# ubc-vision/RefTR

Measured on AMD Instinct MI355X. Metric: images/sec training step, RefCOCO R50 640x640 bs=8/GPU, higher is better.
Workload: dtype bf16; 1 GPU; RefCOCO-shaped REC train step, ResNet-50 + BERT-base + VL transformer 6+6, 640x640, batch 8/GPU, L=40, aux loss, dropout on, clip 0.1, AdamW (configs[1]); global_batch=8, batch_per_gpu=8, image_size=640, parallelism=dp1, launch=hipgraph

## Files before the change

reftr_amd/csrc/rt_qregion.hip:

```cpp
#include "rt_common.h"
#include "rt_ln_row.h"
#include "rt_loss_row.h"

namespace {

constexpr int QE = 256;
constexpr int QT = 1024;
constexpr int QH = QT / 256;
constexpr int QW = QT / 64;

__device__ __forceinline__ f32x4 ld4(const float* p) { return *reinterpret_cast<const f32x4*>(p); }
__device__ __forceinline__ void st4(float* p, const f32x4 v) { *reinterpret_cast<f32x4*>(p) = v; }
__device__ __forceinline__ void st4b(bf16_t* p, const f32x4 v) {
    bf16x4 b;
#pragma unroll
    for (int e = 0; e < 4; ++e) b[e] = (bf16_t)v[e];
    *reinterpret_cast<bf16x4*>(p) = b;
}

template <int MT, int K, typename XRow, typename Epi>
__device__ __forceinline__ void q_tile(const bf16_t* __restrict__ W, const int ldw, const int n0, const int nmax,
                                       XRow xrow, const int M, Epi epi) {
    const int lane = threadIdx.x & 63, li = lane & 15, lg = lane >> 4;
    int n = n0 + li; if (n >= nmax) n = nmax - 1;
    const bf16_t* wp = W + (size_t)n * ldw + lg * 8;
    const bf16_t* xp[MT];
    f32x4 acc[MT];
#pragma unroll
    for (int t = 0; t < MT; ++t) {
        int m = t * 16 + li; if (m >= M) m = M - 1;
        xp[t] = xrow(m) + lg * 8;
        acc[t] = f32x4{0.f, 0.f, 0.f, 0.f};
    }
    constexpr int KC = MT >= 3 ? 128 : (K < 256 ? K : 256), NK = KC / 32;
#pragma unroll
    for (int k0 = 0; k0 < K; k0 += KC) {
        bf16x8 a[NK], x[MT][NK];
#pragma unroll
        for (int i = 0; i < NK; ++i) a[i] = *reinterpret_cast<const bf16x8*>(wp + k0 + i * 32);
#pragma unroll
        for (int t = 0; t < MT; ++t)
#pragma unroll
            for (int i = 0; i < NK; ++i) x[t][i] = *reinterpret_cast<const bf16x8*>(xp[t] + k0 + i * 32);
        __builtin_amdgcn_sched_barrier(0);
#pragma unroll
        for (int i = 0; i < NK; ++i)
#pragma unroll
            for (int t = 0; t < MT; ++t)
                acc[t] = __builtin_amdgcn_mfma_f32_16x16x32_bf16(a[i], x[t][i], acc[t], 0, 0, 0);
        __builtin_amdgcn_sched_barrier(0);
    }
#pragma unroll
    for (int t = 0; t < MT; ++t) {
        const int m = t * 16 + li;
        if (m < M && n0 + lg * 4 < nmax) epi(m, n0 + lg * 4, acc[t]);
    }
}
constexpr int QLMAX = 96;
constexpr int QLD = QE + 8;
__device__ unsigned long long g_qtrace[3][24];
__device__ __forceinline__ void q_stamp(const int kernel, int& slot) {
    if (blockIdx.x == 0 && threadIdx.x == 0 && slot < 24) g_qtrace[kernel][slot] = __builtin_amdgcn_s_memrealtime();
    ++slot;
}
template <int K, typename Epi>
__device__ __forceinline__ void q_tile_lds(const bf16_t* __restrict__ W, const int ldw, const int n0, const int nmax,
                                           const bf16_t* Xs, const int ldx, const int M, const float* __restrict__ bias, Epi epi) {
    const int lane = threadIdx.x & 63, li = lane & 15, lg = lane >> 4;
    int n = n0 + li; if (n >= nmax) n = nmax - 1;
    const bf16_t* wp = W + (size_t)n * ldw + lg * 8;
    constexpr int NK = K / 32;
    bf16x8 a[NK];
#pragma unroll
    for (int i = 0; i < NK; ++i) a[i] = *reinterpret_cast<const bf16x8*>(wp + i * 32);
    const bool nok = n0 + lg * 4 < nmax;
    const f32x4 b4 = (bias && nok) ? ld4(bias + n0 + lg * 4) : f32x4{0.f, 0.f, 0.f, 0.f};
    for (int m0 = 0; m0 < M; m0 += 16) {
        int m = m0 + li; if (m >= M) m = M - 1;
        const bf16_t* xp = Xs + (size_t)m * ldx + lg * 8;
        f32x4 acc = f32x4{0.f, 0.f, 0.f, 0.f};
#pragma unroll
        for (int i = 0; i < NK; ++i)
            acc = __builtin_amdgcn_mfma_f32_16x16x32_bf16(a[i], *reinterpret_cast<const bf16x8*>(xp + i * 32), acc, 0, 0, 0);
        if (m0 + li < M && nok) epi(m0 + li, n0 + lg * 4, acc + b4);
    }
}
template <int K, typename XRow, typename Epi>
__device__ __forceinline__ void q_gemm(const bf16_t* __restrict__ W, const int ldw, const int N, XRow xrow, const int M, Epi epi,
                                       const int tile0 = 0, const int tile_stride = QW) {
    const int wave = threadIdx.x >> 6;
    const int ntiles = (N + 15) >> 4;
    for (int t = tile0 + wave; t < ntiles; t += tile_stride) {
        for (int m0 = 0; m0 < M; m0 += 48) {
            const int rows = min(48, M - m0);
            auto xr = [&](int m) { return xrow(m0 + m); };
            auto ep = [&](int m, int n, const f32x4& v) { epi(m0 + m, n, v); };
            if (rows <= 16)      q_tile<1, K>(W, ldw, t * 16, N, xr, rows, ep);
            else if (rows <= 32) q_tile<2, K>(W, ldw, t * 16, N, xr, rows, ep);
            else                 q_tile<3, K>(W, ldw, t * 16, N, xr, rows, ep);
        }
    }
}

__device__ __forceinline__ f32x4 q_ln(const float* x, const float* gamma, const float* beta, const float eps, const bool relu,
                                      float* mean_out, float* rstd_out) {
    const int lane = threadIdx.x & 63;
    const f32x4 v = ld4(x + lane * 4);
    float mean, rstd;
    rt_ln_stats<1>(&v, eps, mean, rstd);
    if (lane == 0) { *mean_out = mean; *rstd_out = rstd; }
    return rt_ln_affine(v, mean, rstd, ld4(gamma + lane * 4), ld4(beta + lane * 4), relu);
}
__device__ __forceinline__ f32x4 q_ln_bwd(const f32x4 d, const float* x, const float mean, const float rstd, const f32x4 gam, const f32x4 bet,
                                          const bool relu, f32x4& dg, f32x4& db) {
    f32x4 xh, g;
    float s1 = 0.f, s2 = 0.f;
    rt_ln_bwd_group(d, ld4(x + (threadIdx.x & 63) * 4), mean, rstd, gam, bet, relu, xh, g, s1, s2, dg, db);
    rt_ln_bwd_means<1>(s1, s2);
    return rt_ln_bwd_dx(g, xh, rstd, s1, s2);
}
__device__ __forceinline__ void ln_partials(float (*sm)[QE], const f32x4 dg, const f32x4 db, float* __restrict__ part) {
    const int lane = threadIdx.x & 63, wave = threadIdx.x >> 6;
    __syncthreads();
    st4(&sm[wave][lane * 4], dg); st4(&sm[QW + wave][lane * 4], db);
    __syncthreads();
    for (int c = threadIdx.x; c < 2 * QE; c += QT) {
        const int which = c / QE, col = c - which * QE;
        float a = 0.f;
#pragma unroll
        for (int w = 0; w < QW; ++w) a += sm[which * QW + w][col];
        part[((size_t)blockIdx.x * 2 + which) * QE + col] = a;
    }
}

__global__ __launch_bounds__(QT) void qenc_fwd_kernel(const rt_qenc_fwd_desc p) {
    int q_slot = 0; q_stamp(0, q_slot);
    __shared__ float sw[128];
    __shared__ float pw[128];
    __shared__ __attribute__((aligned(16))) bf16_t xs[QLMAX * QLD];
    __shared__ __attribute__((aligned(16))) float part[4][QE];
    const int b = blockIdx.x, lane = threadIdx.x & 63, wave = threadIdx.x >> 6;
    const int S = p.S, L = p.L, P = p.P;
    const bf16_t* mem16 = (const bf16_t*)p.mem16 + (size_t)b * S * QE;
    bf16_t* cls16 = (bf16_t*)p.cls16 + (size_t)b * QE;
    bf16_t* lang16 = (bf16_t*)p.lang16 + (size_t)b * L * QE;
    float* kq = p.kq + (size_t)b * QE;
    float* qs = p.qs + (size_t)b * L * QE;
    float* vs = p.vs + (size_t)b * L * QE;

    for (int i = threadIdx.x; i < L * (QE / 8); i += QT) {
        const int r = i / (QE / 8), c = (i % (QE / 8)) * 8;
        const bf16x8 v = *reinterpret_cast<const bf16x8*>(mem16 + (size_t)r * QE + c);
        *reinterpret_cast<bf16x8*>(xs + (size_t)r * QLD + c) = v;
        *reinterpret_cast<bf16x8*>(lang16 + (size_t)r * QE + c) = v;
        if (r == 0) *reinterpret_cast<bf16x8*>(cls16 + c) = v;
    }
    __syncthreads(); q_stamp(0, q_slot);
    for (int job = wave; job < 48; job += QW) {
        const int prod = job >> 4, t = job & 15;
        if (prod == 0)
            q_tile_lds<QE>((const bf16_t*)p.W1, QE, t * 16, QE, xs, QLD, 1, p.b1, [&](int, int n, const f32x4& v) { st4(kq + n, v); });
        else {
            float* out = prod == 1 ? qs : vs;
            q_tile_lds<QE>((const bf16_t*)(prod == 1 ? p.W2 : p.W3), QE, t * 16, QE, xs, QLD, L, prod == 1 ? p.b2 : p.b3,
                           [&](int m, int n, const f32x4& v) { st4(out + (size_t)m * QE + n, v); });
        }
    }
    __syncthreads(); q_stamp(0, q_slot);

    for (int l = wave; l < L; l += QW) {
        float s = 0.f;
        for (int d = lane; d < QE; d += 64) s += kq[d] * qs[(size_t)l * QE + d];
        s = rt_wave_sum(s);
        if (lane == 0) sw[l] = s;
    }
    __syncthreads(); q_stamp(0, q_slot);
    for (int j = 0; j < P; ++j) {
        const int r = b * P + j;
        const uint8_t* cm = p.ctx + (size_t)r * L;
        if (wave == 0) {
            const float s0 = lane < L ? (cm[lane] ? -INFINITY : sw[lane]) : -INFINITY;
            const float s1 = lane + 64 < L ? (cm[lane + 64] ? -INFINITY : sw[lane + 64]) : -INFINITY;
            const float m = rt_wave_max(fmaxf(s0, s1));
            const float e0 = lane < L ? __expf(s0 - m) : 0.f, e1 = lane + 64 < L ? __expf(s1 - m) : 0.f;
            const float tot = rt_wave_sum(e0) + rt_wave_sum(e1);
            const float inv = 1.f / tot;
            if (lane < L) { pw[lane] = e0 * inv; p.qw[(size_t)r * L + lane] = e0 * inv; }
            if (lane + 64 < L) { pw[lane + 64] = e1 * inv; p.qw[(size_t)r * L + lane + 64] = e1 * inv; }
        }
        __syncthreads();
        {
            const int qt = threadIdx.x >> 8, d = threadIdx.x & 255;
            const int per = (L + 3) >> 2, l0 = qt * per, l1 = min(L, l0 + per);
            float a = 0.f;
            for (int l = l0; l < l1; ++l) a += pw[l] * vs[(size_t)l * QE + d];
            part[qt][d] = a;
        }
        __syncthreads();
        if (threadIdx.x < QE) {
            const int d = threadIdx.x;
            ((bf16_t*)p.c16)[(size_t)r * QE + d] = (bf16_t)((part[0][d] + part[1][d]) + (part[2][d] + part[3][d]));
        }
        __syncthreads();
    }

    {
        const bf16_t* c16 = (const bf16_t*)p.c16 + (size_t)b * P * QE;
        float* co = p.co + (size_t)b * P * QE;
        const float* bc = p.bc;
        q_gemm<QE>((const bf16_t*)p.Wc, QE, QE, [&](int m) { return c16 + (size_t)m * QE; }, P,
                   [&](int m, int n, const f32x4& v) { st4(co + (size_t)m * QE + n, v + ld4(bc + n)); });
    }
    __syncthreads(); q_stamp(0, q_slot);
    bf16_t* cat16 = (bf16_t*)p.cat16;
    for (int j = wave; j < P; j += QW) {
        const int r = b * P + j;
        const f32x4 y = q_ln(p.co + (size_t)r * QE, p.gc, p.betc, p.eps, false, p.cmean + r, p.crstd + r);
        st4b(cat16 + (size_t)r * 2 * QE + lane * 4, y + ld4(p.mem32 + (size_t)b * S * QE + lane * 4));
    }
    __syncthreads(); q_stamp(0, q_slot);
    {
        const float* bf0 = p.bf0;
        q_gemm<2 * QE>((const bf16_t*)p.Wf0, 2 * QE, QE, [&](int m) { return cat16 + (size_t)(b * P + m) * 2 * QE; }, P,
                       [&](int m, int n, const f32x4& v) { st4(p.t1 + (size_t)(b * P + m) * QE + n, v + ld4(bf0 + n)); });
    }
    __syncthreads(); q_stamp(0, q_slot);
    {
        const rt_drop drop = rt_drop::site(p.drop_p, p.seed_dev, p.drop_seed);
        for (int j = wave; j < P; j += QW) {
            const int r = b * P + j;
            f32x4 y = q_ln(p.t1 + (size_t)r * QE, p.g1, p.bet1, p.eps, true, p.m1 + r, p.r1 + r);
            y = drop.apply(y, (uint32_t)(r * QE + lane * 4));
            st4b((bf16_t*)p.a16 + (size_t)r * QE + lane * 4, y);
        }
    }
    __syncthreads(); q_stamp(0, q_slot);
    {
        const bf16_t* a16 = (const bf16_t*)p.a16;
        const float* bf4 = p.bf4;
        q_gemm<QE>((const bf16_t*)p.Wf4, QE, QE, [&](int m) { return a16 + (size_t)(b * P + m) * QE; }, P,
                   [&](int m, int n, const f32x4& v) { st4(p.t2 + (size_t)(b * P + m) * QE + n, v + ld4(bf4 + n)); });
    }
    __syncthreads(); q_stamp(0, q_slot);
    for (int j = wave; j < P; j += QW) {
        const int r = b * P + j;
        const f32x4 f = q_ln(p.t2 + (size_t)r * QE, p.g5, p.bet5, p.eps, true, p.m2 + r, p.r2 + r);
        for (int q = 0; q < p.nq; ++q) {
            const size_t o = ((size_t)r * p.nq + q) * QE + lane * 4;
            const f32x4 tg = f + ld4(p.qembed + (size_t)q * 2 * QE + lane * 4);
            const f32x4 qp = f + ld4(p.qembed + (size_t)q * 2 * QE + QE + lane * 4);
            st4(p.tgt32 + o, tg); st4(p.qpos + o, qp);
            st4b((bf16_t*)p.tgt16 + o, tg); st4b((bf16_t*)p.tgtq16 + o, tg + qp);
        }
    }
    q_stamp(0, q_slot);
}

__global__ __launch_bounds__(QT) void head_loss_kernel(const rt_head_loss_desc p) {
    int q_slot = 0; q_stamp(1, q_slot);
    __shared__ __attribute__((aligned(16))) float sm[2 * QW][QE];
    __shared__ float red[QW][6];
    const int l = blockIdx.x, lane = threadIdx.x & 63, wave = threadIdx.x >> 6;
    const int N = p.B * p.P * p.K;
    const size_t r0 = (size_t)l * N;
    const float* t3 = p.t3 + r0 * QE;
    bf16_t* hs16 = (bf16_t*)p.hs16 + r0 * QE;
    bf16_t* y1 = (bf16_t*)p.y1 + r0 * QE;
    bf16_t* y2 = (bf16_t*)p.y2 + r0 * QE;
    bf16_t* dy2 = (bf16_t*)p.dy2 + r0 * QE;
    bf16_t* dy1 = (bf16_t*)p.dy1 + r0 * QE;
    float* dhs = p.dhs + r0 * QE;

    for (int m = wave; m < N; m += QW) {
        const f32x4 y = q_ln(t3 + (size_t)m * QE, p.gn, p.betn, p.eps, false, p.hmean + r0 + m, p.hrstd + r0 + m);
        st4b(hs16 + (size_t)m * QE + lane * 4, y);
    }
    __syncthreads(); q_stamp(1, q_slot);
    {
        const float* b0 = p.b0;
        q_gemm<QE>((const bf16_t*)p.W0, QE, QE, [&](int m) { return hs16 + (size_t)m * QE; }, N, [&](int m, int n, const f32x4& v) {
            f32x4 y = v + ld4(b0 + n);
#pragma unroll
            for (int e = 0; e < 4; ++e) y[e] = fmaxf(y[e], 0.f);
            st4b(y1 + (size_t)m * QE + n, y);
        });
    }
    __syncthreads(); q_stamp(1, q_slot);
    {
        const float* b1 = p.b1;
        q_gemm<QE>((const bf16_t*)p.W1, QE, QE, [&](int m) { return y1 + (size_t)m * QE; }, N, [&](int m, int n, const f32x4& v) {
            f32x4 y = v + ld4(b1 + n);
#pragma unroll
            for (int e = 0; e < 4; ++e) y[e] = fmaxf(y[e], 0.f);
            st4b(y2 + (size_t)m * QE + n, y);
        });
    }
    __syncthreads(); q_stamp(1, q_slot);
    float l1_sum = 0.f, gi_sum = 0.f, dbias[4] = {0.f, 0.f, 0.f, 0.f};
    {
        const float nb = fmaxf(p.num_boxes[0], 1.f) * (float)p.K;
        const float wb = p.weights[l * 2], wg = p.weights[l * 2 + 1];
        const f32x4 b2 = ld4(p.b2);
        for (int m0 = wave * 48; m0 < N; m0 += QW * 48) {
            const int rows = min(48, N - m0);
            auto xr = [&](int m) { return y2 + (size_t)(m0 + m) * QE; };
            auto ep = [&](int mm, int n, const f32x4& v) {
                if (n != 0) return;
                const int m = m0 + mm;
                const f32x4 lg4 = v + b2;
                st4(p.logits + (r0 + m) * 4, lg4);
                const int k = m % p.K, ph = (m / p.K) % p.P, bi = m / (p.K * p.P);
                f32x4 g4 = f32x4{0.f, 0.f, 0.f, 0.f};
                if ((p.valid[(size_t)bi * p.P * p.K + ph * p.K + k] != 0) != (p.invert_valid != 0)) {
                    int rank = 0, nvalid = 0;
                    for (int q = 0; q < p.P; ++q) {
                        const int vv = ((p.valid[(size_t)bi * p.P * p.K + q * p.K] != 0) != (p.invert_valid != 0)) ? 1 : 0;
                        nvalid += vv;
                        if (q < ph) rank += vv;
                    }
                    const int count = p.tgt_off[bi + 1] - p.tgt_off[bi];
                    const bool mismatch = nvalid != count;
                    const float lg[4] = {lg4[0], lg4[1], lg4[2], lg4[3]};
                    const float* tg = mismatch ? lg : p.targets + ((size_t)p.tgt_off[bi] + rank) * 4;
                    if (mismatch) l1_sum = __builtin_nanf("");
                    float g[4];
                    rt_box_loss_row(lg, tg, wb, wg, nb, l1_sum, gi_sum, g);
                    g4 = f32x4{g[0], g[1], g[2], g[3]};
                }
                st4(p.dlogits + (r0 + m) * 4, g4);
                st4b((bf16_t*)p.dl16 + (r0 + m) * 4, g4);
#pragma unroll
                for (int e = 0; e < 4; ++e) dbias[e] += g4[e];
            };
            if (rows <= 16)      q_tile<1, QE>((const bf16_t*)p.W2, QE, 0, 4, xr, rows, ep);
            else if (rows <= 32) q_tile<2, QE>((const bf16_t*)p.W2, QE, 0, 4, xr, rows, ep);
            else                 q_tile<3, QE>((const bf16_t*)p.W2, QE, 0, 4, xr, rows, ep);
        }
        l1_sum = rt_wave_sum(l1_sum); gi_sum = rt_wave_sum(gi_sum);
#pragma unroll
        for (int e = 0; e < 4; ++e) dbias[e] = rt_wave_sum(dbias[e]);
        if (lane == 0) {
            red[wave][0] = l1_sum; red[wave][1] = gi_sum;
#pragma unroll
            for (int e = 0; e < 4; ++e) red[wave][2 + e] = dbias[e];
        }
        __syncthreads();
        if (threadIdx.x < 6) {
            float a = 0.f;
#pragma unroll
            for (int w = 0; w < QW; ++w) a += red[w][threadIdx.x];
            if (threadIdx.x < 2) {
                __hip_atomic_store(p.losses + l * 2 + threadIdx.x, a / nb, __ATOMIC_RELAXED, __HIP_MEMORY_SCOPE_AGENT);
            } else if (p.db2_part) {
                p.db2_part[l * 8 + (threadIdx.x - 2)] = a; p.db2_part[l * 8 + 4 + (threadIdx.x - 2)] = 0.f;
            }
        }
    }
    if (p.total && p.ticket && threadIdx.x == 0) {
        const int old = __hip_atomic_fetch_add(p.ticket, 1, __ATOMIC_ACQ_REL, __HIP_MEMORY_SCOPE_AGENT);
        if (old == p.NL - 1) {
            float tot = 0.f;
            for (int i = 0; i < p.NL; ++i) {
                const float lb = __hip_atomic_load(p.losses + i * 2, __ATOMIC_RELAXED, __HIP_MEMORY_SCOPE_AGENT);
                const float lg2 = __hip_atomic_load(p.losses + i * 2 + 1, __ATOMIC_RELAXED, __HIP_MEMORY_SCOPE_AGENT);
                tot += p.weights[i * 2] * lb + p.weights[i * 2 + 1] * lg2;
            }
            p.total[0] = tot;
            __hip_atomic_store(p.ticket, 0, __ATOMIC_RELAXED, __HIP_MEMORY_SCOPE_AGENT);
        }
    }
    __syncthreads(); q_stamp(1, q_slot);
    {
        const float* dl = p.dlogits + r0 * 4;
        for (int i = threadIdx.x; i < N * (QE / 4); i += QT) {
            const int m = i / (QE / 4), k = (i % (QE / 4)) * 4;
            const f32x4 d = ld4(dl + (size_t)m * 4);
            const bf16x4 gt = *reinterpret_cast<const bf16x4*>(y2 + (size_t)m * QE + k);
            f32x4 a;
#pragma unroll
            for (int e = 0; e < 4; ++e) {
                float s = 0.f;
#pragma unroll
                for (int n = 0; n < 4; ++n) s += d[n] * p.w2_f32[(size_t)n * QE + k + e];
                a[e] = ((float)gt[e] > 0.f) ? s : 0.f;
            }
            st4b(dy2 + (size_t)m * QE + k, a);
        }
    }
    __syncthreads(); q_stamp(1, q_slot);
    {
        q_gemm<QE>((const bf16_t*)p.W1T, QE, QE, [&](int m) { return dy2 + (size_t)m * QE; }, N, [&](int m, int n, const f32x4& v) {
            const bf16x4 gt = *reinterpret_cast<const bf16x4*>(y1 + (size_t)m * QE + n);
            f32x4 y;
#pragma unroll
            for (int e = 0; e < 4; ++e) y[e] = ((float)gt[e] > 0.f) ? v[e] : 0.f;
            st4b(dy1 + (size_t)m * QE + n, y);
        });
    }
    __syncthreads(); q_stamp(1, q_slot);
    q_gemm<QE>((const bf16_t*)p.W0T, QE, QE, [&](int m) { return dy1 + (size_t)m * QE; }, N,
               [&](int m, int n, const f32x4& v) { st4(dhs + (size_t)m * QE + n, v); });
    __syncthreads(); q_stamp(1, q_slot);
    f32x4 dg = f32x4{0.f, 0.f, 0.f, 0.f}, db = dg;
    {
        const f32x4 gam = ld4(p.gn + lane * 4), bet = ld4(p.betn + lane * 4);
        for (int m = wave; m < N; m += QW) {
            const f32x4 dx = q_ln_bwd(ld4(dhs + (size_t)m * QE + lane * 4), t3 + (size_t)m * QE, p.hmean[r0 + m], p.hrstd[r0 + m], gam, bet,
                                      false, dg, db);
            st4(p.dnorm + (r0 + m) * QE + lane * 4, dx);
        }
    }
    ln_partials(sm, dg, db, p.part_n);
    q_stamp(1, q_slot);
}

__global__ __launch_bounds__(QT) void qenc_bwd_kernel(const rt_qenc_bwd_desc p) {
    int q_slot = 0; q_stamp(2, q_slot);
    __shared__ __attribute__((aligned(16))) float sm[2 * QW][QE];
    __shared__ float sds[16][128];
    __shared__ __attribute__((aligned(16))) bf16_t xdq[QLMAX * QLD], xdv[QLMAX * QLD], xk[QLD];
    __shared__ __attribute__((aligned(16))) float srow[QE];
    const int b = blockIdx.x, lane = threadIdx.x & 63, wave = threadIdx.x >> 6;
    const int S = p.S, L = p.L, P = p.P;
    const int rb = b * P;
    const rt_drop drop = rt_drop::site(p.drop_p, p.seed_dev, p.drop_seed);

    {
        f32x4 dg = f32x4{0.f, 0.f, 0.f, 0.f}, db = dg, sa = dg, sq = dg;
        const f32x4 gam = ld4(p.g5 + lane * 4), bet = ld4(p.bet5 + lane * 4);
        for (int j = wave; j < P; j += QW) {
            const int r = rb + j;
            const f32x4 a = ld4(p.ga + (size_t)r * QE + lane * 4), q = ld4(p.dqpos + (size_t)r * QE + lane * 4);
            f32x4 d = a;
            if (p.gb) { const f32x4 g2 = ld4(p.gb + (size_t)r * QE + lane * 4); d = d + g2; sa = sa + g2; }
            d = d + q;
            sa = sa + a; sq = sq + q;
            const f32x4 dx = q_ln_bwd(d, p.t2 + (size_t)r * QE, p.m2[r], p.r2[r], gam, bet, true, dg, db);
            st4b((bf16_t*)p.dt2b + (size_t)r * QE + lane * 4, dx);
        }
        if (p.dqembed) {
#pragma unroll
            for (int e = 0; e < 4; ++e) {
                if (sa[e] != 0.f) atomicAdd(p.dqembed + lane * 4 + e, sa[e]);
                if (sq[e] != 0.f) atomicAdd(p.dqembed + QE + lane * 4 + e, sq[e]);
            }
        }
        ln_partials(sm, dg, db, p.part5);
    }
    __syncthreads(); q_stamp(2, q_slot);
    q_gemm<QE>((const bf16_t*)p.Wf4T, QE, QE, [&](int m) { return (const bf16_t*)p.dt2b + (size_t)(rb + m) * QE; }, P,
               [&](int m, int n, const f32x4& v) { st4(p.da + (size_t)(rb + m) * QE + n, v); });
    __syncthreads(); q_stamp(2, q_slot);
    {
        f32x4 dg = f32x4{0.f, 0.f, 0.f, 0.f}, db = dg;
        const f32x4 gam = ld4(p.g1 + lane * 4), bet = ld4(p.bet1 + lane * 4);
        for (int j = wave; j < P; j += QW) {
            const int r = rb + j;
            f32x4 d = ld4(p.da + (size_t)r * QE + lane * 4);
            d = drop.apply(d, (uint32_t)(r * QE + lane * 4));
            const f32x4 dx = q_ln_bwd(d, p.t1 + (size_t)r * QE, p.m1[r], p.r1[r], gam, bet, true, dg, db);
            st4b((bf16_t*)p.dt1b + (size_t)r * QE + lane * 4, dx);
        }
        ln_partials(sm, dg, db, p.part1);
    }
    __syncthreads(); q_stamp(2, q_slot);
    q_gemm<QE>((const bf16_t*)p.Wf0T, QE, 2 * QE, [&](int m) { return (const bf16_t*)p.dt1b + (size_t)(rb + m) * QE; }, P,
               [&](int m, int n, const f32x4& v) { st4(p.dcat + (size_t)(rb + m) * 2 * QE + n, v); });
    __syncthreads(); q_stamp(2, q_slot);
    {
        f32x4 dg = f32x4{0.f, 0.f, 0.f, 0.f}, db = dg;
        const f32x4 gam = ld4(p.gc + lane * 4), bet = ld4(p.betc + lane * 4);
        for (int j = wave; j < P; j += QW) {
            const int r = rb + j;
            const f32x4 dx = q_ln_bwd(ld4(p.dcat + (size_t)r * 2 * QE + lane * 4), p.co + (size_t)r * QE, p.cmean[r], p.crstd[r], gam, bet, false, dg, db);
            st4b((bf16_t*)p.dcob + (size_t)r * QE + lane * 4, dx);
        }
        ln_partials(sm, dg, db, p.partc);
        if (threadIdx.x < QE) {
            float a = 0.f;
            for (int j = 0; j < P; ++j) a += p.dcat[(size_t)(rb + j) * 2 * QE + threadIdx.x];
            srow[threadIdx.x] = a;
        }
    }
    __syncthreads(); q_stamp(2, q_slot);
    q_gemm<QE>((const bf16_t*)p.WcT, QE, QE, [&](int m) { return (const bf16_t*)p.dcob + (size_t)(rb + m) * QE; }, P,
               [&](int m, int n, const f32x4& v) { st4(p.dc + (size_t)(rb + m) * QE + n, v); });
    __syncthreads(); q_stamp(2, q_slot);
    {
        const float* qs = p.qs + (size_t)b * L * QE;
        const float* vs = p.vs + (size_t)b * L * QE;
        const float* kq = p.kq + (size_t)b * QE;
        for (int i = wave; i < P * L; i += QW) {
            const int j = i / L, l = i - j * L;
            float s = 0.f;
            for (int d = lane; d < QE; d += 64) s += p.dc[(size_t)(rb + j) * QE + d] * vs[(size_t)l * QE + d];
            s = rt_wave_sum(s);
            if (lane == 0) sds[j][l] = s;
        }
        __syncthreads();
        for (int j = wave; j < P; j += QW) {
            const float* wr = p.qw + (size_t)(rb + j) * L;
            const float w0 = lane < L ? wr[lane] : 0.f, w1 = lane + 64 < L ? wr[lane + 64] : 0.f;
            const float d0 = lane < L ? sds[j][lane] : 0.f, d1 = lane + 64 < L ? sds[j][lane + 64] : 0.f;
            const float dot = rt_wave_sum(w0 * d0) + rt_wave_sum(w1 * d1);
            if (lane < L) sds[j][lane] = w0 * (d0 - dot);
            if (lane + 64 < L) sds[j][lane + 64] = w1 * (d1 - dot);
        }
        __syncthreads();
        const int d = threadIdx.x & 255, hf = threadIdx.x >> 8;
        const float kd = kq[d];
        float gk = 0.f;
        for (int l = hf; l < L; l += QH) {
            float dq = 0.f, dv = 0.f;
            for (int j = 0; j < P; ++j) {
                const float ds = sds[j][l];
                dq += ds * kd;
                dv += p.qw[(size_t)(rb + j) * L + l] * p.dc[(size_t)(rb + j) * QE + d];
                gk += ds * qs[(size_t)l * QE + d];
            }
            ((bf16_t*)p.dqs16)[((size_t)b * L + l) * QE + d] = (bf16_t)dq; xdq[(size_t)l * QLD + d] = (bf16_t)dq;
            ((bf16_t*)p.dvs16)[((size_t)b * L + l) * QE + d] = (bf16_t)dv; xdv[(size_t)l * QLD + d] = (bf16_t)dv;
        }
        sm[hf][d] = gk;
        __syncthreads();
        if (threadIdx.x < QE) {
            const bf16_t v = (bf16_t)((sm[0][d] + sm[1][d]) + (sm[2][d] + sm[3][d]));
            ((bf16_t*)p.dk16)[(size_t)b * QE + d] = v; xk[d] = v;
        }
    }
    __syncthreads(); q_stamp(2, q_slot);
    {
        float* dmem = p.dmem + (size_t)b * S * QE;
        for (int t = wave; t < QE / 16; t += QW) {
            const int lanei = lane & 15;
            f32x4 dcls = f32x4{0.f, 0.f, 0.f, 0.f};
            q_tile_lds<QE>((const bf16_t*)p.W1T, QE, t * 16, QE, xk, QLD, 1, nullptr, [&](int, int, const f32x4& v) { dcls = v; });
            const int lg = lane >> 4;
            const bf16_t* w2p = (const bf16_t*)p.W2T + (size_t)(t * 16 + lanei) * QE + lg * 8;
            const bf16_t* w3p = (const bf16_t*)p.W3T + (size_t)(t * 16 + lanei) * QE + lg * 8;
            bf16x8 a2[QE / 32], a3[QE / 32];
#pragma unroll
            for (int i = 0; i < QE / 32; ++i) { a2[i] = *reinterpret_cast<const bf16x8*>(w2p + i * 32); a3[i] = *reinterpret_cast<const bf16x8*>(w3p + i * 32); }
            for (int m0 = 0; m0 < L; m0 += 16) {
                int m = m0 + lanei; if (m >= L) m = L - 1;
                const bf16_t* xq = xdq + (size_t)m * QLD + lg * 8;
                const bf16_t* xv = xdv + (size_t)m * QLD + lg * 8;
                f32x4 aq = f32x4{0.f, 0.f, 0.f, 0.f}, av = aq;
#pragma unroll
                for (int i = 0; i < QE / 32; ++i) {
                    aq = __builtin_amdgcn_mfma_f32_16x16x32_bf16(a2[i], *reinterpret_cast<const bf16x8*>(xq + i * 32), aq, 0, 0, 0);
                    av = __builtin_amdgcn_mfma_f32_16x16x32_bf16(a3[i], *reinterpret_cast<const bf16x8*>(xv + i * 32), av, 0, 0, 0);
                }
                if (m0 + lanei < L) {
                    float* o = dmem + (size_t)(m0 + lanei) * QE + t * 16 + lg * 4;
                    f32x4 cur = ld4(o);
                    if (m0 + lanei == 0) {
                        cur = cur + ld4(srow + t * 16 + lg * 4);
                        cur = cur + dcls;
                    }
                    st4(o, cur + (av + aq));
                }
            }
        }
    }
    q_stamp(2, q_slot);
}

}

extern "C" int rt_qenc_fwd(const rt_qenc_fwd_desc* d, rt_stream_t stream) {
    if (!d || !d->mem16 || !d->mem32 || !d->ctx || !d->cat16 || !d->tgt32) return RT_ERR_BADARG;
    if (d->E != QE || d->L <= 0 || d->L > QLMAX || d->P <= 0 || d->P > 16 || d->nq <= 0 || d->B <= 0) return RT_ERR_UNSUPPORTED;
    hipLaunchKernelGGL(qenc_fwd_kernel, dim3(d->B), dim3(QT), 0, (hipStream_t)stream, *d);
    RT_CHECK_LAUNCH();
    return RT_OK;
}

extern "C" int rt_head_loss(const rt_head_loss_desc* d, rt_stream_t stream) {
    if (!d || !d->t3 || !d->logits || !d->losses || !d->weights || !d->valid || !d->targets || !d->tgt_off || !d->num_boxes ||
        !d->dnorm || !d->part_n) return RT_ERR_BADARG;
    if (d->E != QE || d->NL <= 0 || d->B <= 0 || d->P <= 0 || d->K <= 0) return RT_ERR_UNSUPPORTED;
    hipLaunchKernelGGL(head_loss_kernel, dim3(d->NL), dim3(QT), 0, (hipStream_t)stream, *d);
    RT_CHECK_LAUNCH();
    return RT_OK;
}

extern "C" int rt_qenc_bwd(const rt_qenc_bwd_desc* d, rt_stream_t stream) {
    if (!d || !d->ga || !d->dqpos || !d->dmem || !d->part5 || !d->part1 || !d->partc) return RT_ERR_BADARG;
    if (d->E != QE || d->L <= 0 || d->L > QLMAX || d->P <= 0 || d->P > 16 || d->B <= 0) return RT_ERR_UNSUPPORTED;
    hipLaunchKernelGGL(qenc_bwd_kernel, dim3(d->B), dim3(QT), 0, (hipStream_t)stream, *d);
    RT_CHECK_LAUNCH();
    return RT_OK;
}

extern "C" int rt_qregion_trace(unsigned long long* host_out) {
    if (!host_out) return RT_ERR_BADARG;
    return (int)hipMemcpyFromSymbol(host_out, HIP_SYMBOL(g_qtrace), sizeof(unsigned long long) * 3 * 24);
}
```

Baseline: 1259 images/s.

## Coalesce weight loads via per-wave LDS staging with swizzled fragment reshuffle

```diff
diff --git a/reftr_amd/csrc/rt_qregion.hip b/reftr_amd/csrc/rt_qregion.hip
--- a/reftr_amd/csrc/rt_qregion.hip
+++ b/reftr_amd/csrc/rt_qregion.hip
@@ -18,12 +18,49 @@
     *reinterpret_cast<bf16x4*>(p) = b;
 }
 
+constexpr int QSTG = 16 * 128;
+__device__ __forceinline__ void q_wave_order() {
+    __builtin_amdgcn_fence(__ATOMIC_ACQ_REL, "wavefront");
+    __builtin_amdgcn_wave_barrier();
+}
+template <int KC>
+__device__ __forceinline__ void q_wreq(const bf16_t* __restrict__ W, const int ldw, const int n0, const int nmax, const int k0,
+                                       bf16x8 (&raw)[KC / 32]) {
+    constexpr int LPR = KC / 8, RPI = 64 / LPR;
+    const int lane = threadIdx.x & 63, q = lane / LPR, c = lane % LPR;
+    int col = k0 + c * 8;
+    asm volatile("" : "+v"(col));
+#pragma unroll
+    for (int j = 0; j < KC / 32; ++j) {
+        const int n = min(n0 + j * RPI + q, nmax - 1);
+        raw[j] = *reinterpret_cast<const bf16x8*>(W + (size_t)n * ldw + col);
+    }
+}
+template <int KC>
+__device__ __forceinline__ void q_wfrag(unsigned char* stg, const bf16x8 (&raw)[KC / 32], bf16x8 (&a)[KC / 32]) {
+    static_assert(KC == 128 || KC == 256, "whole rows per wave instruction, two or four of them");
+    constexpr int LPR = KC / 8, RPI = 64 / LPR;
+    const int lane = threadIdx.x & 63, li = lane & 15, lg = lane >> 4, c = lane % LPR, q = lane / LPR;
+    int wb = q * 128 + (((c & 7) ^ (q >> 1)) << 4), rb = li * 128 + ((lg ^ ((li >> 1) & 7)) << 4);
+    asm volatile("" : "+v"(wb), "+v"(rb));
+#pragma unroll
+    for (int s = 0; s < KC / 64; ++s) {
+        if ((c >> 3) == s) {
+#pragma unroll
+            for (int j = 0; j < KC / 32; ++j)
+                *reinterpret_cast<bf16x8*>(stg + ((wb ^ (((j * RPI / 2) & 7) << 4)) + j * RPI * 128)) = raw[j];
+        }
+        q_wave_order();
+#pragma unroll
+        for (int i = 0; i < 2; ++i) a[2 * s + i] = *reinterpret_cast<const bf16x8*>(stg + (rb ^ (i << 6)));
+        q_wave_order();
+    }
+}
+
 template <int MT, int K, typename XRow, typename Epi>
 __device__ __forceinline__ void q_tile(const bf16_t* __restrict__ W, const int ldw, const int n0, const int nmax,
-                                       XRow xrow, const int M, Epi epi) {
+                                       XRow xrow, const int M, unsigned char* stg, Epi epi) {
     const int lane = threadIdx.x & 63, li = lane & 15, lg = lane >> 4;
-    int n = n0 + li; if (n >= nmax) n = nmax - 1;
-    const bf16_t* wp = W + (size_t)n * ldw + lg * 8;
     const bf16_t* xp[MT];
     f32x4 acc[MT];
 #pragma unroll
@@ -32,17 +69,17 @@
         xp[t] = xrow(m) + lg * 8;
         acc[t] = f32x4{0.f, 0.f, 0.f, 0.f};
     }
-    constexpr int KC = MT >= 3 ? 128 : (K < 256 ? K : 256), NK = KC / 32;
+    constexpr int KC = MT >= 2 ? 128 : (K < 256 ? K : 256), NK = KC / 32;
 #pragma unroll
     for (int k0 = 0; k0 < K; k0 += KC) {
-        bf16x8 a[NK], x[MT][NK];
-#pragma unroll
-        for (int i = 0; i < NK; ++i) a[i] = *reinterpret_cast<const bf16x8*>(wp + k0 + i * 32);
+        bf16x8 raw[NK], a[NK], x[MT][NK];
+        q_wreq<KC>(W, ldw, n0, nmax, k0, raw);
 #pragma unroll
         for (int t = 0; t < MT; ++t)
 #pragma unroll
             for (int i = 0; i < NK; ++i) x[t][i] = *reinterpret_cast<const bf16x8*>(xp[t] + k0 + i * 32);
         __builtin_amdgcn_sched_barrier(0);
+        q_wfrag<KC>(stg, raw, a);
 #pragma unroll
         for (int i = 0; i < NK; ++i)
 #pragma unroll
@@ -65,16 +102,15 @@
 }
 template <int K, typename Epi>
 __device__ __forceinline__ void q_tile_lds(const bf16_t* __restrict__ W, const int ldw, const int n0, const int nmax,
-                                           const bf16_t* Xs, const int ldx, const int M, const float* __restrict__ bias, Epi epi) {
+                                           const bf16_t* Xs, const int ldx, const int M, const float* __restrict__ bias,
+                                           unsigned char* stg, Epi epi) {
     const int lane = threadIdx.x & 63, li = lane & 15, lg = lane >> 4;
-    int n = n0 + li; if (n >= nmax) n = nmax - 1;
-    const bf16_t* wp = W + (size_t)n * ldw + lg * 8;
     constexpr int NK = K / 32;
-    bf16x8 a[NK];
-#pragma unroll
-    for (int i = 0; i < NK; ++i) a[i] = *reinterpret_cast<const bf16x8*>(wp + i * 32);
+    bf16x8 raw[NK], a[NK];
+    q_wreq<K>(W, ldw, n0, nmax, 0, raw);
     const bool nok = n0 + lg * 4 < nmax;
     const f32x4 b4 = (bias && nok) ? ld4(bias + n0 + lg * 4) : f32x4{0.f, 0.f, 0.f, 0.f};
+    q_wfrag<K>(stg, raw, a);
     for (int m0 = 0; m0 < M; m0 += 16) {
         int m = m0 + li; if (m >= M) m = M - 1;
         const bf16_t* xp = Xs + (size_t)m * ldx + lg * 8;
@@ -85,19 +121,21 @@
         if (m0 + li < M && nok) epi(m0 + li, n0 + lg * 4, acc + b4);
     }
 }
-template <int K, typename XRow, typename Epi>
-__device__ __forceinline__ void q_gemm(const bf16_t* __restrict__ W, const int ldw, const int N, XRow xrow, const int M, Epi epi,
-                                       const int tile0 = 0, const int tile_stride = QW) {
+template <int K, int MTMAX, typename XRow, typename Epi>
+__device__ __forceinline__ void q_gemm(const bf16_t* __restrict__ W, const int ldw, const int N, XRow xrow, const int M, unsigned char* wst,
+                                       Epi epi) {
     const int wave = threadIdx.x >> 6;
     const int ntiles = (N + 15) >> 4;
-    for (int t = tile0 + wave; t < ntiles; t += tile_stride) {
-        for (int m0 = 0; m0 < M; m0 += 48) {
-            const int rows = min(48, M - m0);
+    unsigned char* stg = wst + wave * QSTG;
+    for (int t = wave; t < ntiles; t += QW) {
+        if (MTMAX == 1) { q_tile<1, K>(W, ldw, t * 16, N, xrow, M, stg, epi); continue; }
+        for (int m0 = 0; m0 < M; m0 += MTMAX * 16) {
+            const int rows = min(MTMAX * 16, M - m0);
             auto xr = [&](int m) { return xrow(m0 + m); };
             auto ep = [&](int m, int n, const f32x4& v) { epi(m0 + m, n, v); };
-            if (rows <= 16)      q_tile<1, K>(W, ldw, t * 16, N, xr, rows, ep);
-            else if (rows <= 32) q_tile<2, K>(W, ldw, t * 16, N, xr, rows, ep);
-            else                 q_tile<3, K>(W, ldw, t * 16, N, xr, rows, ep);
+            if (rows <= 16)                    q_tile<1, K>(W, ldw, t * 16, N, xr, rows, stg, ep);
+            else if (MTMAX == 2 || rows <= 32) q_tile<2, K>(W, ldw, t * 16, N, xr, rows, stg, ep);
+            else                               q_tile<3, K>(W, ldw, t * 16, N, xr, rows, stg, ep);
         }
     }
 }
@@ -139,6 +177,7 @@
     __shared__ float pw[128];
     __shared__ __attribute__((aligned(16))) bf16_t xs[QLMAX * QLD];
     __shared__ __attribute__((aligned(16))) float part[4][QE];
+    __shared__ __attribute__((aligned(16))) unsigned char wst[QW * QSTG];
     const int b = blockIdx.x, lane = threadIdx.x & 63, wave = threadIdx.x >> 6;
     const int S = p.S, L = p.L, P = p.P;
     const bf16_t* mem16 = (const bf16_t*)p.mem16 + (size_t)b * S * QE;
@@ -159,10 +198,10 @@
     for (int job = wave; job < 48; job += QW) {
         const int prod = job >> 4, t = job & 15;
         if (prod == 0)
-            q_tile_lds<QE>((const bf16_t*)p.W1, QE, t * 16, QE, xs, QLD, 1, p.b1, [&](int, int n, const f32x4& v) { st4(kq + n, v); });
+            q_tile_lds<QE>((const bf16_t*)p.W1, QE, t * 16, QE, xs, QLD, 1, p.b1, wst + wave * QSTG, [&](int, int n, const f32x4& v) { st4(kq + n, v); });
         else {
             float* out = prod == 1 ? qs : vs;
-            q_tile_lds<QE>((const bf16_t*)(prod == 1 ? p.W2 : p.W3), QE, t * 16, QE, xs, QLD, L, prod == 1 ? p.b2 : p.b3,
+            q_tile_lds<QE>((const bf16_t*)(prod == 1 ? p.W2 : p.W3), QE, t * 16, QE, xs, QLD, L, prod == 1 ? p.b2 : p.b3, wst + wave * QSTG,
                            [&](int m, int n, const f32x4& v) { st4(out + (size_t)m * QE + n, v); });
         }
     }
@@ -208,7 +247,7 @@
         const bf16_t* c16 = (const bf16_t*)p.c16 + (size_t)b * P * QE;
         float* co = p.co + (size_t)b * P * QE;
         const float* bc = p.bc;
-        q_gemm<QE>((const bf16_t*)p.Wc, QE, QE, [&](int m) { return c16 + (size_t)m * QE; }, P,
+        q_gemm<QE, 1>((const bf16_t*)p.Wc, QE, QE, [&](int m) { return c16 + (size_t)m * QE; }, P, wst,
                    [&](int m, int n, const f32x4& v) { st4(co + (size_t)m * QE + n, v + ld4(bc + n)); });
     }
     __syncthreads(); q_stamp(0, q_slot);
@@ -221,7 +260,7 @@
     __syncthreads(); q_stamp(0, q_slot);
     {
         const float* bf0 = p.bf0;
-        q_gemm<2 * QE>((const bf16_t*)p.Wf0, 2 * QE, QE, [&](int m) { return cat16 + (size_t)(b * P + m) * 2 * QE; }, P,
+        q_gemm<2 * QE, 1>((const bf16_t*)p.Wf0, 2 * QE, QE, [&](int m) { return cat16 + (size_t)(b * P + m) * 2 * QE; }, P, wst,
                        [&](int m, int n, const f32x4& v) { st4(p.t1 + (size_t)(b * P + m) * QE + n, v + ld4(bf0 + n)); });
     }
     __syncthreads(); q_stamp(0, q_slot);
@@ -238,7 +277,7 @@
     {
         const bf16_t* a16 = (const bf16_t*)p.a16;
         const float* bf4 = p.bf4;
-        q_gemm<QE>((const bf16_t*)p.Wf4, QE, QE, [&](int m) { return a16 + (size_t)(b * P + m) * QE; }, P,
+        q_gemm<QE, 1>((const bf16_t*)p.Wf4, QE, QE, [&](int m) { return a16 + (size_t)(b * P + m) * QE; }, P, wst,
                    [&](int m, int n, const f32x4& v) { st4(p.t2 + (size_t)(b * P + m) * QE + n, v + ld4(bf4 + n)); });
     }
     __syncthreads(); q_stamp(0, q_slot);
@@ -260,6 +299,7 @@
     int q_slot = 0; q_stamp(1, q_slot);
     __shared__ __attribute__((aligned(16))) float sm[2 * QW][QE];
     __shared__ float red[QW][6];
+    __shared__ __attribute__((aligned(16))) unsigned char wst[QW * QSTG];
     const int l = blockIdx.x, lane = threadIdx.x & 63, wave = threadIdx.x >> 6;
     const int N = p.B * p.P * p.K;
     const size_t r0 = (size_t)l * N;
@@ -278,7 +318,7 @@
     __syncthreads(); q_stamp(1, q_slot);
     {
         const float* b0 = p.b0;
-        q_gemm<QE>((const bf16_t*)p.W0, QE, QE, [&](int m) { return hs16 + (size_t)m * QE; }, N, [&](int m, int n, const f32x4& v) {
+        q_gemm<QE, 3>((const bf16_t*)p.W0, QE, QE, [&](int m) { return hs16 + (size_t)m * QE; }, N, wst, [&](int m, int n, const f32x4& v) {
             f32x4 y = v + ld4(b0 + n);
 #pragma unroll
             for (int e = 0; e < 4; ++e) y[e] = fmaxf(y[e], 0.f);
@@ -288,7 +328,7 @@
     __syncthreads(); q_stamp(1, q_slot);
     {
         const float* b1 = p.b1;
-        q_gemm<QE>((const bf16_t*)p.W1, QE, QE, [&](int m) { return y1 + (size_t)m * QE; }, N, [&](int m, int n, const f32x4& v) {
+        q_gemm<QE, 3>((const bf16_t*)p.W1, QE, QE, [&](int m) { return y1 + (size_t)m * QE; }, N, wst, [&](int m, int n, const f32x4& v) {
             f32x4 y = v + ld4(b1 + n);
 #pragma unroll
             for (int e = 0; e < 4; ++e) y[e] = fmaxf(y[e], 0.f);
@@ -332,9 +372,9 @@
 #pragma unroll
                 for (int e = 0; e < 4; ++e) dbias[e] += g4[e];
             };
-            if (rows <= 16)      q_tile<1, QE>((const bf16_t*)p.W2, QE, 0, 4, xr, rows, ep);
-            else if (rows <= 32) q_tile<2, QE>((const bf16_t*)p.W2, QE, 0, 4, xr, rows, ep);
-            else                 q_tile<3, QE>((const bf16_t*)p.W2, QE, 0, 4, xr, rows, ep);
+            if (rows <= 16)      q_tile<1, QE>((const bf16_t*)p.W2, QE, 0, 4, xr, rows, wst + wave * QSTG, ep);
+            else if (rows <= 32) q_tile<2, QE>((const bf16_t*)p.W2, QE, 0, 4, xr, rows, wst + wave * QSTG, ep);
+            else                 q_tile<3, QE>((const bf16_t*)p.W2, QE, 0, 4, xr, rows, wst + wave * QSTG, ep);
         }
         l1_sum = rt_wave_sum(l1_sum); gi_sum = rt_wave_sum(gi_sum);
 #pragma unroll
@@ -389,7 +429,7 @@
     }
     __syncthreads(); q_stamp(1, q_slot);
     {
-        q_gemm<QE>((const bf16_t*)p.W1T, QE, QE, [&](int m) { return dy2 + (size_t)m * QE; }, N, [&](int m, int n, const f32x4& v) {
+        q_gemm<QE, 3>((const bf16_t*)p.W1T, QE, QE, [&](int m) { return dy2 + (size_t)m * QE; }, N, wst, [&](int m, int n, const f32x4& v) {
             const bf16x4 gt = *reinterpret_cast<const bf16x4*>(y1 + (size_t)m * QE + n);
             f32x4 y;
 #pragma unroll
@@ -398,7 +438,7 @@
         });
     }
     __syncthreads(); q_stamp(1, q_slot);
-    q_gemm<QE>((const bf16_t*)p.W0T, QE, QE, [&](int m) { return dy1 + (size_t)m * QE; }, N,
+    q_gemm<QE, 3>((const bf16_t*)p.W0T, QE, QE, [&](int m) { return dy1 + (size_t)m * QE; }, N, wst,
                [&](int m, int n, const f32x4& v) { st4(dhs + (size_t)m * QE + n, v); });
     __syncthreads(); q_stamp(1, q_slot);
     f32x4 dg = f32x4{0.f, 0.f, 0.f, 0.f}, db = dg;
@@ -420,6 +460,8 @@
     __shared__ float sds[16][128];
     __shared__ __attribute__((aligned(16))) bf16_t xdq[QLMAX * QLD], xdv[QLMAX * QLD], xk[QLD];
     __shared__ __attribute__((aligned(16))) float srow[QE];
+    static_assert(sizeof(sm) >= QW * QSTG, "staging regions alias sm");
+    unsigned char* wst = reinterpret_cast<unsigned char*>(&sm[0][0]);
     const int b = blockIdx.x, lane = threadIdx.x & 63, wave = threadIdx.x >> 6;
     const int S = p.S, L = p.L, P = p.P;
     const int rb = b * P;
@@ -448,7 +490,7 @@
         ln_partials(sm, dg, db, p.part5);
     }
     __syncthreads(); q_stamp(2, q_slot);
-    q_gemm<QE>((const bf16_t*)p.Wf4T, QE, QE, [&](int m) { return (const bf16_t*)p.dt2b + (size_t)(rb + m) * QE; }, P,
+    q_gemm<QE, 1>((const bf16_t*)p.Wf4T, QE, QE, [&](int m) { return (const bf16_t*)p.dt2b + (size_t)(rb + m) * QE; }, P, wst,
                [&](int m, int n, const f32x4& v) { st4(p.da + (size_t)(rb + m) * QE + n, v); });
     __syncthreads(); q_stamp(2, q_slot);
     {
@@ -464,7 +506,7 @@
         ln_partials(sm, dg, db, p.part1);
     }
     __syncthreads(); q_stamp(2, q_slot);
-    q_gemm<QE>((const bf16_t*)p.Wf0T, QE, 2 * QE, [&](int m) { return (const bf16_t*)p.dt1b + (size_t)(rb + m) * QE; }, P,
+    q_gemm<QE, 1>((const bf16_t*)p.Wf0T, QE, 2 * QE, [&](int m) { return (const bf16_t*)p.dt1b + (size_t)(rb + m) * QE; }, P, wst,
                [&](int m, int n, const f32x4& v) { st4(p.dcat + (size_t)(rb + m) * 2 * QE + n, v); });
     __syncthreads(); q_stamp(2, q_slot);
     {
@@ -483,7 +525,7 @@
         }
     }
     __syncthreads(); q_stamp(2, q_slot);
-    q_gemm<QE>((const bf16_t*)p.WcT, QE, QE, [&](int m) { return (const bf16_t*)p.dcob + (size_t)(rb + m) * QE; }, P,
+    q_gemm<QE, 1>((const bf16_t*)p.WcT, QE, QE, [&](int m) { return (const bf16_t*)p.dcob + (size_t)(rb + m) * QE; }, P, wst,
                [&](int m, int n, const f32x4& v) { st4(p.dc + (size_t)(rb + m) * QE + n, v); });
     __syncthreads(); q_stamp(2, q_slot);
     {
@@ -534,13 +576,13 @@
         for (int t = wave; t < QE / 16; t += QW) {
             const int lanei = lane & 15;
             f32x4 dcls = f32x4{0.f, 0.f, 0.f, 0.f};
-            q_tile_lds<QE>((const bf16_t*)p.W1T, QE, t * 16, QE, xk, QLD, 1, nullptr, [&](int, int, const f32x4& v) { dcls = v; });
+            q_tile_lds<QE>((const bf16_t*)p.W1T, QE, t * 16, QE, xk, QLD, 1, nullptr, wst + wave * QSTG, [&](int, int, const f32x4& v) { dcls = v; });
             const int lg = lane >> 4;
-            const bf16_t* w2p = (const bf16_t*)p.W2T + (size_t)(t * 16 + lanei) * QE + lg * 8;
-            const bf16_t* w3p = (const bf16_t*)p.W3T + (size_t)(t * 16 + lanei) * QE + lg * 8;
-            bf16x8 a2[QE / 32], a3[QE / 32];
-#pragma unroll
-            for (int i = 0; i < QE / 32; ++i) { a2[i] = *reinterpret_cast<const bf16x8*>(w2p + i * 32); a3[i] = *reinterpret_cast<const bf16x8*>(w3p + i * 32); }
+            bf16x8 r2[QE / 32], r3[QE / 32], a2[QE / 32], a3[QE / 32];
+            q_wreq<QE>((const bf16_t*)p.W2T, QE, t * 16, QE, 0, r2);
+            q_wreq<QE>((const bf16_t*)p.W3T, QE, t * 16, QE, 0, r3);
+            q_wfrag<QE>(wst + wave * QSTG, r2, a2);
+            q_wfrag<QE>(wst + wave * QSTG, r3, a3);
             for (int m0 = 0; m0 < L; m0 += 16) {
                 int m = m0 + lanei; if (m >= L) m = L - 1;
                 const bf16_t* xq = xdq + (size_t)m * QLD + lg * 8;
```

After: 1255 images/s, median of 2. About the same (-0.3%).
